# heitorrapela/HalluciDet

Measured on AMD Instinct MI355X. Metric: images/sec train_hallucidet (640x512, batch 8/GPU), higher is better.
Workload: dtype f16; 1 GPU; train_hallucidet.py fasterrcnn LLVIP batch=8 fp16 on 1xMI355X (BASELINE configs[1]); U-Net resnet34 fwd+bwd, 3 frozen Faster R-CNN R50-FPN passes @300x300 (one batched evaluation of 24 images: trunk, RPN, RoI heads, NMS for all three; the RGB / IR passes' LOSS VALUES, which the reference computes and discards, are not evaluated), loss scaling, value clip 0.5, Adam; global_batch=8, image=1x512x640 IR + 3x512x640 RGB, batch_per_gpu=8, parallelism=dp1

## Files before the change

hallucidet_amd/csrc/detection.hip:

```cpp
#include "hd_common.h"
#pragma clang fp contract(off)

namespace {

__device__ __forceinline__ float box_iou_dev(const float* a, const float* b) {
  float area_a = (a[2] - a[0]) * (a[3] - a[1]);
  float area_b = (b[2] - b[0]) * (b[3] - b[1]);
  float xx1 = fmaxf(a[0], b[0]), yy1 = fmaxf(a[1], b[1]);
  float xx2 = fminf(a[2], b[2]), yy2 = fminf(a[3], b[3]);
  float w = fmaxf(0.f, xx2 - xx1), h = fmaxf(0.f, yy2 - yy1);
  float inter = w * h;
  return inter / (area_a + area_b - inter);
}

__global__ void nms_mask_kernel(const float* __restrict__ boxes, const int* __restrict__ counts, int nmax, float thr,
                                uint64_t* __restrict__ mask) {
  const int b = blockIdx.z;
  const int n = counts[b];
  const int row0 = blockIdx.y * 64, col0 = blockIdx.x * 64;
  if (row0 >= n || col0 >= n || blockIdx.x < blockIdx.y) return;
  const int cb = (nmax + 63) / 64;
  __shared__ float cbx[64 * 4];
  const float* bb = boxes + (size_t)b * nmax * 4;
  int t = threadIdx.x;
  int ncol = min(64, n - col0);
  if (t < ncol) {
    cbx[t * 4 + 0] = bb[(col0 + t) * 4 + 0];
    cbx[t * 4 + 1] = bb[(col0 + t) * 4 + 1];
    cbx[t * 4 + 2] = bb[(col0 + t) * 4 + 2];
    cbx[t * 4 + 3] = bb[(col0 + t) * 4 + 3];
  }
  __syncthreads();
  int i = row0 + t;
  if (i < n) {
    float me[4] = {bb[i * 4], bb[i * 4 + 1], bb[i * 4 + 2], bb[i * 4 + 3]};
    uint64_t m = 0;
    int start = (row0 == col0) ? t + 1 : 0;
    for (int j = start; j < ncol; ++j)
      if (box_iou_dev(me, cbx + j * 4) > thr) m |= (1ull << j);
    mask[((size_t)b * nmax + i) * cb + blockIdx.x] = m;
  }
}

__global__ __launch_bounds__(256) void nms_reduce_kernel(const uint64_t* __restrict__ mask, const int* __restrict__ counts, int nmax,
                                                         uint8_t* __restrict__ keep, int max_keep, const int64_t* __restrict__ order,
                                                         int64_t* __restrict__ pick, int pick_n, int64_t* __restrict__ picked) {
  constexpr int MAXW = 4;
  __shared__ uint64_t remv[MAXW * 64];
  __shared__ uint64_t part[4][MAXW * 64];
  __shared__ uint64_t s_keepbits;
  __shared__ int s_kept;
  const int b = blockIdx.x;
  const int n = counts[b];
  const int cb = (nmax + 63) / 64;
  const int tid = threadIdx.x, lane = tid & 63, wave = tid >> 6;
  const uint64_t* mb = mask + (size_t)b * nmax * cb;
  uint8_t* kb = keep + (size_t)b * nmax;
  const int nchunks = (n + 63) / 64;
  for (int i = tid; i < MAXW * 64; i += 256) remv[i] = 0;
  if (tid == 0) s_kept = 0;
  if (pick)
    for (int i = tid; i < pick_n; i += 256) pick[(size_t)b * pick_n + i] = order[(size_t)b * nmax];
  __syncthreads();
  for (int c = 0; c < nchunks; ++c) {
    if (s_kept >= max_keep) {
      for (int i = c * 64 + tid; i < n; i += 256) kb[i] = 0;
      break;
    }
    const int lim = min(64, n - c * 64);
    if (wave == 0) {
      const int i = c * 64 + lane;
      const uint64_t diag = (i < n) ? mb[(size_t)i * cb + c] : 0;
      const unsigned dlo = (unsigned)diag, dhi = (unsigned)(diag >> 32);
      uint64_t alive = ~remv[c];
      if (lim < 64) alive &= (1ull << lim) - 1ull;
      alive = ((uint64_t)(unsigned)__builtin_amdgcn_readfirstlane((unsigned)(alive >> 32)) << 32) |
              (uint64_t)(unsigned)__builtin_amdgcn_readfirstlane((unsigned)alive);
      uint64_t keepbits = 0;
      for (int it = 0; it < 64 && alive; ++it) {
        const int j = __builtin_amdgcn_readfirstlane(__builtin_ctzll(alive));
        keepbits |= (1ull << j);
        const uint64_t dj = ((uint64_t)(unsigned)__builtin_amdgcn_readlane(dhi, j) << 32) | (uint64_t)(unsigned)__builtin_amdgcn_readlane(dlo, j);
        alive &= ~dj;
        alive &= ~(1ull << j);
      }
      if (i < n) kb[i] = (uint8_t)((keepbits >> lane) & 1ull);
      if (pick && ((keepbits >> lane) & 1ull)) {
        const int pos = s_kept + __popcll(keepbits & ((1ull << lane) - 1ull));
        if (pos < pick_n) pick[(size_t)b * pick_n + pos] = order[(size_t)b * nmax + i];
      }
      if (lane == 0) {
        s_keepbits = keepbits;
        s_kept += __popcll(keepbits);
      }
    }
    __syncthreads();
    const uint64_t keepbits = s_keepbits;
    const int nw = nchunks - (c + 1);
    if (nw > 0) {
      for (int wb = 0; wb < nw; wb += 64) {
        const int w = c + 1 + wb + lane;
        const bool act = w < nchunks;
        uint64_t accw = 0;
        for (int jb = wave * 16; jb < lim; jb += 64) {
          uint64_t rws[16];
#pragma unroll
          for (int u = 0; u < 16; ++u) {
            const int j = min(jb + u, lim - 1);
            rws[u] = act ? mb[(size_t)(c * 64 + j) * cb + w] : 0ull;
          }
#pragma unroll
          for (int u = 0; u < 16; ++u)
            if (jb + u < lim && ((keepbits >> (jb + u)) & 1ull)) accw |= rws[u];
        }
        part[wave][wb + lane] = accw;
      }
      __syncthreads();
      for (int i = tid; i < nw; i += 256) remv[c + 1 + i] |= part[0][i] | part[1][i] | part[2][i] | part[3][i];
    }
    __syncthreads();
  }
  if (picked && tid == 0) picked[b] = min(s_kept, pick_n);
}

__global__ __launch_bounds__(256) void nms_prepare_kernel(const float* __restrict__ boxes, const int64_t* __restrict__ idxs,
                                                          const uint8_t* __restrict__ valid, const int64_t* __restrict__ order, int n,
                                                          float* __restrict__ sorted, int* __restrict__ counts) {
  __shared__ float s_max[4];
  __shared__ int s_cnt[4];
  const int b = blockIdx.x, tid = threadIdx.x;
  const float* bb = boxes + (size_t)b * n * 4;
  const uint8_t* vb = valid + (size_t)b * n;
  float m = -INFINITY;
  int cnt = 0;
  for (int i = tid; i < n; i += 256)
    if (vb[i]) {
      const float4 v = *reinterpret_cast<const float4*>(bb + (size_t)i * 4);
      m = fmaxf(fmaxf(m, fmaxf(v.x, v.y)), fmaxf(v.z, v.w));
      ++cnt;
    }
#pragma unroll
  for (int d = 32; d >= 1; d >>= 1) {
    m = fmaxf(m, __shfl_xor(m, d));
    cnt += __shfl_xor(cnt, d);
  }
  if ((tid & 63) == 0) {
    s_max[tid >> 6] = m;
    s_cnt[tid >> 6] = cnt;
  }
  __syncthreads();
  cnt = s_cnt[0] + s_cnt[1] + s_cnt[2] + s_cnt[3];
  m = fmaxf(fmaxf(s_max[0], s_max[1]), fmaxf(s_max[2], s_max[3]));
  const float scale = (cnt > 0 ? m : 0.f) + 1.f;
  if (tid == 0) counts[b] = cnt;
  for (int j = tid; j < n; j += 256) {
    const int64_t c = order[(size_t)b * n + j];
    const float off = (float)idxs[(size_t)b * n + c] * scale;
    float4 v = *reinterpret_cast<const float4*>(bb + (size_t)c * 4);
    v.x += off; v.y += off; v.z += off; v.w += off;
    *reinterpret_cast<float4*>(sorted + ((size_t)b * n + j) * 4) = v;
  }
}

struct NmsSegs {
  int off[9];
  int L, S;
};

__global__ __launch_bounds__(256) void nms_seg_prepare_kernel(const float* __restrict__ boxes, const uint8_t* __restrict__ valid, int n, NmsSegs sg,
                                                              float* __restrict__ sorted, int64_t* __restrict__ order, int* __restrict__ counts) {
  __shared__ float s_max[4];
  __shared__ int s_cnt[4];
  __shared__ int s_wsum[4];
  const int b = blockIdx.x, tid = threadIdx.x, lane = tid & 63, wave = tid >> 6;
  const float* bb = boxes + (size_t)b * n * 4;
  const uint8_t* vb = valid + (size_t)b * n;
  float m = -INFINITY;
  int cnt = 0;
  for (int i = tid; i < n; i += 256)
    if (vb[i]) {
      const float4 v = *reinterpret_cast<const float4*>(bb + (size_t)i * 4);
      m = fmaxf(fmaxf(m, fmaxf(v.x, v.y)), fmaxf(v.z, v.w));
      ++cnt;
    }
#pragma unroll
  for (int d = 32; d >= 1; d >>= 1) {
    m = fmaxf(m, __shfl_xor(m, d));
    cnt += __shfl_xor(cnt, d);
  }
  if (lane == 0) {
    s_max[wave] = m;
    s_cnt[wave] = cnt;
  }
  __syncthreads();
  cnt = s_cnt[0] + s_cnt[1] + s_cnt[2] + s_cnt[3];
  m = fmaxf(fmaxf(s_max[0], s_max[1]), fmaxf(s_max[2], s_max[3]));
  const float scale = (cnt > 0 ? m : 0.f) + 1.f;
  for (int l = 0; l < sg.L; ++l) {
    const int lo = sg.off[l], hi = sg.off[l + 1];
    const float off = (float)l * scale;
    float* so = sorted + ((size_t)b * sg.L + l) * sg.S * 4;
    int64_t* oo = order + ((size_t)b * sg.L + l) * sg.S;
    int base = 0;
    for (int c0 = lo; c0 < hi; c0 += 256) {
      const int i = c0 + tid;
      const bool v = i < hi && vb[i];
      const uint64_t bal = __ballot(v);
      const int before = __popcll(bal & ((1ull << lane) - 1ull));
      __syncthreads();
      if (lane == 0) s_wsum[wave] = __popcll(bal);
      __syncthreads();
      int wbase = 0;
      for (int w = 0; w < wave; ++w) wbase += s_wsum[w];
      if (v) {
        const int r = base + wbase + before;
        float4 bx = *reinterpret_cast<const float4*>(bb + (size_t)i * 4);
        bx.x += off; bx.y += off; bx.z += off; bx.w += off;
        *reinterpret_cast<float4*>(so + (size_t)r * 4) = bx;
        oo[r] = i;
      }
      base += s_wsum[0] + s_wsum[1] + s_wsum[2] + s_wsum[3];
    }
    if (tid == 0) counts[b * sg.L + l] = base;
  }
}

__global__ __launch_bounds__(256) void nms_seg_merge_kernel(const float* __restrict__ scores, const int64_t* __restrict__ pick_seg,
                                                            const int64_t* __restrict__ picked_seg, int n, int pick_n_seg, NmsSegs sg, int top_k,
                                                            int64_t* __restrict__ pick, int64_t* __restrict__ picked) {
  extern __shared__ float s_sc[];
  const int b = blockIdx.x / sg.L, l = blockIdx.x % sg.L;
  const float* sb = scores + (size_t)b * n;
  int cnt[8], total = 0;
  for (int q = 0; q < sg.L; ++q) {
    cnt[q] = (int)picked_seg[b * sg.L + q];
    total += cnt[q];
    const int64_t* pq = pick_seg + ((size_t)b * sg.L + q) * pick_n_seg;
    for (int r = threadIdx.x; r < cnt[q]; r += 256) s_sc[q * pick_n_seg + r] = sb[pq[r]];
  }
  __syncthreads();
  const int64_t* pk = pick_seg + (size_t)blockIdx.x * pick_n_seg;
  for (int r = threadIdx.x; r < cnt[l]; r += 256) {
    const float sc = s_sc[l * pick_n_seg + r];
    int rank = r;
    for (int q = 0; q < sg.L; ++q) {
      if (q == l) continue;
      const float* a = s_sc + q * pick_n_seg;
      int lo = 0, hi = cnt[q];
      if (q < l) {
        while (lo < hi) { const int mid = (lo + hi) >> 1; if (a[mid] >= sc) lo = mid + 1; else hi = mid; }
      } else {
        while (lo < hi) { const int mid = (lo + hi) >> 1; if (a[mid] > sc) lo = mid + 1; else hi = mid; }
      }
      rank += lo;
    }
    if (rank < top_k) pick[(size_t)b * top_k + rank] = pk[r];
  }
  if (l == 0) {
    int64_t best = 0;
    float bs = -INFINITY;
    bool any = false;
    for (int q = 0; q < sg.L; ++q)
      if (cnt[q] > 0 && (!any || s_sc[q * pick_n_seg] > bs)) {
        any = true;
        bs = s_sc[q * pick_n_seg];
        best = pick_seg[((size_t)b * sg.L + q) * pick_n_seg];
      }
    const int have = total < top_k ? total : top_k;
    for (int r = have + threadIdx.x; r < top_k; r += 256) pick[(size_t)b * top_k + r] = best;
    if (threadIdx.x == 0) picked[b] = have;
  }
}

__global__ void box_iou_kernel(const float* __restrict__ gt, int G, const float* __restrict__ boxes, int A, float* __restrict__ iou) {
  const int64_t total = (int64_t)G * A;
  for (int64_t i = (int64_t)blockIdx.x * blockDim.x + threadIdx.x; i < total; i += (int64_t)gridDim.x * blockDim.x) {
    int a = (int)(i % A), g = (int)(i / A);
    iou[i] = box_iou_dev(gt + g * 4, boxes + (size_t)a * 4);
  }
}

__global__ void box_iou_batched_kernel(const float* __restrict__ gt, int G, const float* __restrict__ boxes, int A, int N,
                                       long boxes_stride, float* __restrict__ iou) {
  const int64_t total = (int64_t)N * G * A;
  for (int64_t i = (int64_t)blockIdx.x * blockDim.x + threadIdx.x; i < total; i += (int64_t)gridDim.x * blockDim.x) {
    int a = (int)(i % A);
    int64_t q = i / A;
    int g = (int)(q % G);
    int n = (int)(q / G);
    iou[i] = box_iou_dev(gt + ((size_t)n * G + g) * 4, boxes + (size_t)n * boxes_stride + (size_t)a * 4);
  }
}


template <bool DESC>
__device__ __forceinline__ void radix_find_digit(const int* hist, int remaining, uint32_t prefix, int shift, uint32_t* s_prefix,
                                                 int* s_remaining) {
  if (threadIdx.x >= 64) return;
  const int l = threadIdx.x;
  int h[4], tot = 0;
#pragma unroll
  for (int j = 0; j < 4; ++j) {
    h[j] = hist[DESC ? 255 - (4 * l + j) : 4 * l + j];
    tot += h[j];
  }
  int incl = tot;
#pragma unroll
  for (int d = 1; d < 64; d <<= 1) {
    const int t = __shfl_up(incl, d);
    if (l >= d) incl += t;
  }
  const int excl = incl - tot;
  const bool hit = excl < remaining && remaining <= incl;
  const bool fallback = l == 63 && incl < remaining;
  if (hit || fallback) {
    int cum = excl, j = 0;
    for (; j < 3; ++j) {
      if (cum + h[j] >= remaining) break;
      cum += h[j];
    }
    const int bin = DESC ? 255 - (4 * l + j) : 4 * l + j;
    *s_prefix = prefix | ((uint32_t)bin << shift);
    *s_remaining = remaining - cum;
  }
}

__device__ __forceinline__ uint32_t order_key(float f) {
  if (f != f) return 0xFFFFFFFFu;
  uint32_t u = __float_as_uint(f == 0.f ? 0.f : f);
  return (u & 0x80000000u) ? ~u : (u | 0x80000000u);
}

struct TopkSegs {
  int nseg;
  int seg_off[8], n[8], k[8], out_off[8];
};

__global__ __launch_bounds__(1024) void topk_select_kernel(const float* __restrict__ scores, long row_stride, TopkSegs segs,
                                                           int64_t* __restrict__ out, long out_stride) {
  const int seg_off = segs.seg_off[blockIdx.y], n = segs.n[blockIdx.y], k = segs.k[blockIdx.y], out_off = segs.out_off[blockIdx.y];
  const int64_t idx_add = seg_off;
  __shared__ int hist[256];
  __shared__ uint32_t s_prefix;
  __shared__ int s_remaining;
  __shared__ int s_wave_g[16], s_wave_e[16];
  __shared__ uint64_t s_pair[4096];
  const int tid = threadIdx.x, lane = tid & 63, wave = tid >> 6;
  const float* row = scores + (size_t)blockIdx.x * row_stride + seg_off;
  int64_t* orow = out + (size_t)blockIdx.x * out_stride + out_off;
  int P = 1;
  while (P < k) P <<= 1;
  if (k >= n) {
    for (int i = tid; i < n; i += 1024) s_pair[i] = ((uint64_t)order_key(row[i]) << 32) | (uint32_t)~i;
  } else {
    uint32_t prefix = 0, mask = 0;
    int remaining = k;
    for (int pass = 0; pass < 4; ++pass) {
      const int shift = 24 - 8 * pass;
      if (tid < 256) hist[tid] = 0;
      __syncthreads();
      for (int i = tid; i < n; i += 1024) {
        const uint32_t u = order_key(row[i]);
        if ((u & mask) == prefix) atomicAdd(&hist[(u >> shift) & 255], 1);
      }
      __syncthreads();
      radix_find_digit<true>(hist, remaining, prefix, shift, &s_prefix, &s_remaining);
      __syncthreads();
      prefix = s_prefix;
      remaining = s_remaining;
      mask |= 255u << shift;
      __syncthreads();
    }
    const uint32_t T = prefix;
    int base_g = 0, base_e = 0;
    for (int i0 = 0; i0 < n; i0 += 1024) {
      const int i = i0 + tid;
      const uint32_t u = i < n ? order_key(row[i]) : 0u;
      const bool gt = i < n && u > T, eq = i < n && u == T;
      const uint64_t bg = __ballot(gt), be = __ballot(eq);
      const uint64_t below = (1ull << lane) - 1ull;
      if (lane == 0) {
        s_wave_g[wave] = __popcll(bg);
        s_wave_e[wave] = __popcll(be);
      }
      __syncthreads();
      int g_before = base_g + __popcll(bg & below), e_before = base_e + __popcll(be & below);
      int tot_g = 0, tot_e = 0;
#pragma unroll
      for (int w = 0; w < 16; ++w) {
        if (w < wave) {
          g_before += s_wave_g[w];
          e_before += s_wave_e[w];
        }
        tot_g += s_wave_g[w];
        tot_e += s_wave_e[w];
      }
      if (gt || (eq && e_before < remaining)) s_pair[g_before + min(e_before, remaining)] = ((uint64_t)u << 32) | (uint32_t)~i;
      base_g += tot_g;
      base_e += tot_e;
      __syncthreads();
    }
  }
  for (int i = k + tid; i < P; i += 1024) s_pair[i] = 0;
  __syncthreads();
  for (int size = 2; size <= P; size <<= 1) {
    for (int stride = size >> 1; stride > 0; stride >>= 1) {
      for (int t = tid; t < (P >> 1); t += 1024) {
        const int lo = 2 * t - (t & (stride - 1));
        const int hi = lo + stride;
        const bool desc = (lo & size) == 0;
        const uint64_t a = s_pair[lo], b = s_pair[hi];
        if ((a < b) == desc) {
          s_pair[lo] = b;
          s_pair[hi] = a;
        }
      }
      __syncthreads();
    }
  }
  for (int i = tid; i < k; i += 1024) orow[i] = (int64_t)(uint32_t)~(uint32_t)s_pair[i] + idx_add;
}

__device__ __forceinline__ float4 decode_clip_dev(const float* c, const float* b, float iwx, float iwy, float iww, float iwh, float xclip,
                                                  float img_h, float img_w) {
  const float w = b[2] - b[0], h = b[3] - b[1];
  const float cx = b[0] + 0.5f * w, cy = b[1] + 0.5f * h;
  const float dx = c[0] * iwx, dy = c[1] * iwy;
  float dw = c[2] * iww, dh = c[3] * iwh;
  dw = dw > xclip ? xclip : dw;
  dh = dh > xclip ? xclip : dh;
  const float pcx = dx * w + cx, pcy = dy * h + cy;
  const float pw = expf(dw) * w, ph = expf(dh) * h;
  float4 o;
  o.x = pcx - 0.5f * pw;
  o.y = pcy - 0.5f * ph;
  o.z = pcx + 0.5f * pw;
  o.w = pcy + 0.5f * ph;
  o.x = o.x < 0.f ? 0.f : (o.x > img_w ? img_w : o.x);
  o.z = o.z < 0.f ? 0.f : (o.z > img_w ? img_w : o.z);
  o.y = o.y < 0.f ? 0.f : (o.y > img_h ? img_h : o.y);
  o.w = o.w < 0.f ? 0.f : (o.w > img_h ? img_h : o.w);
  return o;
}

__global__ void rpn_decode_filter_kernel(const float* __restrict__ deltas, const float* __restrict__ obj, const float* __restrict__ anchors,
                                         const int64_t* __restrict__ top, int N, int A, int K, float xclip, float img_h, float img_w,
                                         float min_size, float score_thresh, float* __restrict__ boxes, float* __restrict__ prob,
                                         uint8_t* __restrict__ valid) {
  const int j = blockIdx.x * blockDim.x + threadIdx.x;
  if (j >= N * K) return;
  const int n = j / K;
  const int64_t a = top[j];
  const float4 o = decode_clip_dev(deltas + ((size_t)n * A + a) * 4, anchors + (size_t)a * 4, 1.f, 1.f, 1.f, 1.f, xclip, img_h, img_w);
  const float x = obj[(size_t)n * A + a];
  const float p = 1.f / (1.f + expf(-x));
  *reinterpret_cast<float4*>(boxes + (size_t)j * 4) = o;
  prob[j] = p;
  valid[j] = ((o.z - o.x) >= min_size) && ((o.w - o.y) >= min_size) && (p >= score_thresh);
}

__global__ void roi_decode_clip_kernel(const float* __restrict__ codes, const float* __restrict__ rois, long roi_stride, int R, int K,
                                       float wx, float wy, float ww, float wh, float xclip, float img_h, float img_w,
                                       float* __restrict__ boxes) {
  const int j = blockIdx.x * blockDim.x + threadIdx.x;
  if (j >= R * K) return;
  const int r = j / K;
  *reinterpret_cast<float4*>(boxes + (size_t)j * 4) = decode_clip_dev(codes + (size_t)j * 4, rois + (size_t)r * roi_stride, wx, wy, ww, wh, xclip,
                                                                      img_h, img_w);
}

__global__ void roi_postprocess_kernel(const float* __restrict__ logits, const float* __restrict__ codes, const float* __restrict__ rois,
                                       long roi_stride, const int64_t* __restrict__ counts, int R, int C, int S, float wx, float wy, float ww,
                                       float wh, float xclip, float img_h, float img_w, float score_thresh, float min_size,
                                       float* __restrict__ boxes, float* __restrict__ scores, uint8_t* __restrict__ valid) {
  const int K = C - 1;
  const int j = blockIdx.x * blockDim.x + threadIdx.x;
  if (j >= R * K) return;
  const int r = j / K, k = j - r * K + 1;
  const bool real = (r % S) < (int)counts[r / S];
  float4 o = make_float4(0.f, 0.f, 0.f, 0.f);
  float p = 0.f;
  bool v = false;
  if (real) {
    const float* lr = logits + (size_t)r * C;
    float mx = lr[0];
    for (int c = 1; c < C; ++c) mx = fmaxf(mx, lr[c]);
    float se = 0.f;
    for (int c = 0; c < C; ++c) se += expf(lr[c] - mx);
    p = expf(lr[k] - mx) / se;
    o = decode_clip_dev(codes + ((size_t)r * C + k) * 4, rois + (size_t)r * roi_stride, wx, wy, ww, wh, xclip, img_h, img_w);
    v = (p > score_thresh) && ((o.z - o.x) >= min_size) && ((o.w - o.y) >= min_size);
  }
  *reinterpret_cast<float4*>(boxes + (size_t)j * 4) = o;
  scores[j] = p;
  valid[j] = v;
}

__global__ void roi_samples_finish_kernel(const int64_t* __restrict__ sel, int R, const float* __restrict__ comb, const int64_t* __restrict__ lab,
                                          const int64_t* __restrict__ matched, const float* __restrict__ gt, const uint8_t* __restrict__ gvalid,
                                          int T, int G, float wx, float wy, float ww, float wh, float* __restrict__ rois,
                                          int64_t* __restrict__ labels, float* __restrict__ reg_t) {
  const int r = blockIdx.x * blockDim.x + threadIdx.x;
  if (r >= R) return;
  const int64_t s = sel[r];
  if (s < 0) {
    rois[(size_t)r * 5 + 0] = (float)(-s - 1);
    rois[(size_t)r * 5 + 1] = rois[(size_t)r * 5 + 2] = rois[(size_t)r * 5 + 3] = rois[(size_t)r * 5 + 4] = 0.f;
    labels[r] = -1;
    *reinterpret_cast<float4*>(reg_t + (size_t)r * 4) = make_float4(0.f, 0.f, 0.f, 0.f);
    return;
  }
  const int n = (int)(s / T);
  const float4 b = *reinterpret_cast<const float4*>(comb + (size_t)s * 4);
  bool has_gt = false;
  for (int g = 0; g < G; ++g) has_gt = has_gt || gvalid[(size_t)n * G + g];
  const int64_t m = matched[s];
  float4 rg = make_float4(0.f, 0.f, 0.f, 0.f);
  if (has_gt) rg = *reinterpret_cast<const float4*>(gt + ((size_t)n * G + (m > 0 ? m : 0)) * 4);
  rois[(size_t)r * 5 + 0] = (float)n;
  rois[(size_t)r * 5 + 1] = b.x;
  rois[(size_t)r * 5 + 2] = b.y;
  rois[(size_t)r * 5 + 3] = b.z;
  rois[(size_t)r * 5 + 4] = b.w;
  labels[r] = lab[s];
  const float ew = b.z - b.x, eh = b.w - b.y;
  const float ecx = b.x + 0.5f * ew, ecy = b.y + 0.5f * eh;
  const float gw = rg.z - rg.x, gh = rg.w - rg.y;
  const float gcx = rg.x + 0.5f * gw, gcy = rg.y + 0.5f * gh;
  float4 t;
  t.x = wx * (gcx - ecx) / ew;
// ... 115 lines not shown
    const int i = i0 + tid;
    const bool mem = i < A && member(i);
    const uint32_t u = mem ? key_of(i) : 0xFFFFFFFFu;
    const bool lt = mem && u < T, eq = mem && u == T;
    const uint64_t be = __ballot(eq);
    if (lane == 0) s_wave_e[wave] = __popcll(be);
    __syncthreads();
    int e_before = base_e + __popcll(be & ((1ull << lane) - 1ull));
    int tot_e = 0;
#pragma unroll
    for (int w = 0; w < 16; ++w) {
      if (w < wave) e_before += s_wave_e[w];
      tot_e += s_wave_e[w];
    }
    if (i < A) out[i] = (lt || (eq && e_before < remaining)) ? 1 : 0;
    base_e += tot_e;
    __syncthreads();
  }
}

__global__ __launch_bounds__(1024) void sample_pos_neg_kernel(const int64_t* __restrict__ labels, const int32_t* __restrict__ keys, int A,
                                                              int batch_size, int cap_pos, uint8_t* __restrict__ pos_sel,
                                                              uint8_t* __restrict__ neg_sel, int64_t* __restrict__ counts, int use_lds) {
  __shared__ int hist[256];
  __shared__ uint32_t s_prefix;
  __shared__ int s_remaining;
  __shared__ int s_wave_l[16], s_wave_e[16];
  __shared__ int s_P, s_N;
  extern __shared__ uint32_t s_dyn[];
  const int n = blockIdx.x, tid = threadIdx.x;
  const int64_t* lb = labels + (size_t)n * A;
  const int32_t* kb = keys + (size_t)n * A;
  uint32_t* lk = use_lds ? s_dyn : nullptr;
  uint8_t* lc = use_lds ? reinterpret_cast<uint8_t*>(s_dyn + A) : nullptr;
  if (tid == 0) s_P = s_N = 0;
  __syncthreads();
  int p = 0, q = 0;
  for (int i = tid; i < A; i += 1024) {
    const int64_t l = lb[i];
    p += l >= 1;
    q += l == 0;
    if (use_lds) {
      lk[i] = (uint32_t)kb[i];
      lc[i] = l >= 1 ? 1 : (l == 0 ? 0 : 2);
    }
  }
#pragma unroll
  for (int d = 32; d >= 1; d >>= 1) {
    p += __shfl_xor(p, d);
    q += __shfl_xor(q, d);
  }
  if ((tid & 63) == 0) {
    atomicAdd(&s_P, p);
    atomicAdd(&s_N, q);
  }
  __syncthreads();
  const int P = s_P, Nn = s_N;
  const int num_pos = min(P, cap_pos);
  const int num_neg = min(Nn, batch_size - num_pos);
  if (tid == 0) {
    counts[(size_t)n * 2 + 0] = num_pos;
    counts[(size_t)n * 2 + 1] = num_neg;
  }
  select_smallest_marked(kb, lb, A, true, num_pos, P, pos_sel + (size_t)n * A, hist, &s_prefix, &s_remaining, s_wave_l, s_wave_e, lk, lc);
  __syncthreads();
  select_smallest_marked(kb, lb, A, false, num_neg, Nn, neg_sel + (size_t)n * A, hist, &s_prefix, &s_remaining, s_wave_l, s_wave_e, lk, lc);
}


__global__ __launch_bounds__(1024) void match_best_kernel(const float* __restrict__ gt, const uint8_t* __restrict__ gvalid, int G,
                                                          const float* __restrict__ boxes, int A, long boxes_stride,
                                                          float* __restrict__ best) {
  const int ng = blockIdx.x;
  const int n = ng / G;
  __shared__ float red[16];
  float m = -1.f;
  if (gvalid[ng]) {
    const float g4[4] = {gt[(size_t)ng * 4 + 0], gt[(size_t)ng * 4 + 1], gt[(size_t)ng * 4 + 2], gt[(size_t)ng * 4 + 3]};
    const float* bb = boxes + (size_t)n * boxes_stride;
    for (int a = threadIdx.x; a < A; a += 1024) m = fmaxf(m, box_iou_dev(g4, bb + (size_t)a * 4));
  }
#pragma unroll
  for (int d = 32; d >= 1; d >>= 1) m = fmaxf(m, __shfl_xor(m, d));
  if ((threadIdx.x & 63) == 0) red[threadIdx.x >> 6] = m;
  __syncthreads();
  if (threadIdx.x == 0) {
    float r = red[0];
#pragma unroll
    for (int w = 1; w < 16; ++w) r = fmaxf(r, red[w]);
    best[ng] = r;
  }
}

__global__ __launch_bounds__(256) void match_assign_kernel(const float* __restrict__ gt, const uint8_t* __restrict__ gvalid,
                                                           const int64_t* __restrict__ glabels, int G, const float* __restrict__ boxes,
                                                           int A, int N, long boxes_stride, float high, float low,
                                                           const float* __restrict__ best, float wx, float wy, float ww, float wh,
                                                           int want_reg, int64_t* __restrict__ matched, int64_t* __restrict__ labels,
                                                           float* __restrict__ reg_t) {
  extern __shared__ float s_gt[];
  const int n = blockIdx.y;
  float* s_best = s_gt + G * 4;
  float* s_valid = s_best + G;
  for (int i = threadIdx.x; i < G * 4; i += 256) s_gt[i] = gt[(size_t)n * G * 4 + i];
  for (int i = threadIdx.x; i < G; i += 256) {
    s_best[i] = best ? best[n * G + i] : 0.f;
    s_valid[i] = gvalid[n * G + i] ? 1.f : 0.f;
  }
  __syncthreads();
  const int a = blockIdx.x * 256 + threadIdx.x;
  if (a >= A) return;
  const float* bp = boxes + (size_t)n * boxes_stride + (size_t)a * 4;
  const float b4[4] = {bp[0], bp[1], bp[2], bp[3]};
  float vmax = -INFINITY;
  int imax = 0;
  bool is_best = false, has_gt = false;
  for (int g = 0; g < G; ++g) {
    const bool v = s_valid[g] != 0.f;
    has_gt = has_gt || v;
    const float iou = v ? box_iou_dev(s_gt + g * 4, b4) : -1.f;
    if (iou > vmax) {
      vmax = iou;
      imax = g;
    }
    if (best && v && iou == s_best[g]) is_best = true;
  }
  int64_t m = imax;
  if (vmax < low) m = -1;
  else if (vmax < high) m = -2;
  if (is_best) m = imax;
  const size_t o = (size_t)n * A + a;
  matched[o] = m;
  if (labels) {
    int64_t lab = m >= 0 ? (glabels ? glabels[(size_t)n * G + m] : 1) : (m == -1 ? 0 : -1);
    labels[o] = has_gt ? lab : 0;
  }
  if (want_reg) {
    const float* r = s_gt + (m > 0 ? (int)m : 0) * 4;
    const float ew = b4[2] - b4[0], eh = b4[3] - b4[1];
    const float ecx = b4[0] + 0.5f * ew, ecy = b4[1] + 0.5f * eh;
    const float gw = r[2] - r[0], gh = r[3] - r[1];
    const float gcx = r[0] + 0.5f * gw, gcy = r[1] + 0.5f * gh;
    float4 t;
    t.x = wx * (gcx - ecx) / ew;
    t.y = wy * (gcy - ecy) / eh;
    t.z = ww * logf(gw / ew);
    t.w = wh * logf(gh / eh);
    *reinterpret_cast<float4*>(reg_t + o * 4) = t;
  }
}

}

extern "C" int hd_box_iou_batched(const float* gt, int G, const float* boxes, int A, int N, int shared_boxes, float* iou, void* stream) {
  HD_CHECK_ARG(gt && boxes && iou && G >= 0 && A >= 0 && N >= 0, "hd_box_iou_batched: bad args");
  if (G == 0 || A == 0 || N == 0) return HD_OK;
  int64_t total = (int64_t)N * G * A;
  int g = (int)((total + 255) / 256);
  if (g > 8192) g = 8192;
  hipLaunchKernelGGL(box_iou_batched_kernel, dim3(g), dim3(256), 0, (hipStream_t)stream, gt, G, boxes, A, N,
                     shared_boxes ? 0l : (long)A * 4, iou);
  HD_CHECK_LAUNCH();
  return HD_OK;
}


extern "C" int hd_rpn_decode_filter(const float* deltas, const float* objectness, const float* anchors, const int64_t* top, int N, int A, int K,
                                    float bbox_xform_clip, float img_h, float img_w, float min_size, float score_thresh, float* boxes,
                                    float* prob, uint8_t* valid, void* stream) {
  HD_CHECK_ARG(deltas && objectness && anchors && top && boxes && prob && valid && N >= 0 && A >= 0 && K >= 0, "hd_rpn_decode_filter: bad args");
  if (N * K == 0) return HD_OK;
  hipLaunchKernelGGL(rpn_decode_filter_kernel, dim3((N * K + 255) / 256), dim3(256), 0, (hipStream_t)stream, deltas, objectness, anchors, top, N,
                     A, K, bbox_xform_clip, img_h, img_w, min_size, score_thresh, boxes, prob, valid);
  HD_CHECK_LAUNCH();
  return HD_OK;
}

extern "C" int hd_roi_decode_clip(const float* codes, const float* rois, long roi_stride, int R, int K, const float* coder_weights,
                                  float bbox_xform_clip, float img_h, float img_w, float* boxes, void* stream) {
  HD_CHECK_ARG(codes && rois && coder_weights && boxes && R >= 0 && K >= 0 && roi_stride >= 4, "hd_roi_decode_clip: bad args");
  if (R * K == 0) return HD_OK;
  hipLaunchKernelGGL(roi_decode_clip_kernel, dim3((R * K + 255) / 256), dim3(256), 0, (hipStream_t)stream, codes, rois, roi_stride, R, K,
                     1.0f / coder_weights[0], 1.0f / coder_weights[1], 1.0f / coder_weights[2], 1.0f / coder_weights[3], bbox_xform_clip, img_h,
                     img_w, boxes);
  HD_CHECK_LAUNCH();
  return HD_OK;
}

extern "C" int hd_roi_postprocess(const float* class_logits, const float* box_regression, const float* rois, long roi_stride, const int64_t* counts,
                                  int R, int C, int S, const float* coder_weights, float bbox_xform_clip, float img_h, float img_w, float score_thresh,
                                  float min_size, float* boxes, float* scores, uint8_t* valid, void* stream) {
  HD_CHECK_ARG(class_logits && box_regression && rois && counts && coder_weights && boxes && scores && valid && R >= 0 && C >= 2 && S > 0 &&
               roi_stride >= 4, "hd_roi_postprocess: bad args");
  if (R == 0) return HD_OK;
  const int total = R * (C - 1);
  hipLaunchKernelGGL(roi_postprocess_kernel, dim3((total + 255) / 256), dim3(256), 0, (hipStream_t)stream, class_logits, box_regression, rois,
                     roi_stride, counts, R, C, S, 1.0f / coder_weights[0], 1.0f / coder_weights[1], 1.0f / coder_weights[2], 1.0f / coder_weights[3],
                     bbox_xform_clip, img_h, img_w, score_thresh, min_size, boxes, scores, valid);
  HD_CHECK_LAUNCH();
  return HD_OK;
}

extern "C" int hd_roi_samples_finish(const int64_t* sel, int R, const float* comb, const int64_t* lab, const int64_t* matched, const float* gt,
                                     const uint8_t* gvalid, int T, int G, const float* coder_weights, float* rois, int64_t* labels, float* reg_t,
                                     void* stream) {
  HD_CHECK_ARG(R >= 0 && T > 0 && G > 0 && coder_weights, "hd_roi_samples_finish: bad args");
  if (R == 0) return HD_OK;
  HD_CHECK_ARG(sel && comb && lab && matched && gt && gvalid && rois && labels && reg_t, "hd_roi_samples_finish: null pointer");
  hipLaunchKernelGGL(roi_samples_finish_kernel, dim3((R + 255) / 256), dim3(256), 0, (hipStream_t)stream, sel, R, comb, lab, matched, gt, gvalid, T,
                     G, coder_weights[0], coder_weights[1], coder_weights[2], coder_weights[3], rois, labels, reg_t);
  HD_CHECK_LAUNCH();
  return HD_OK;
}

extern "C" int hd_roi_samples_padded(const uint8_t* pos_sel, const uint8_t* neg_sel, const float* comb, const int64_t* lab, const int64_t* matched,
                                     const float* gt, const uint8_t* gvalid, int N, int T, int G, int S, const float* coder_weights, float* rois,
                                     int64_t* labels, float* reg_t, int64_t* counts, void* stream) {
  HD_CHECK_ARG(pos_sel && neg_sel && comb && lab && matched && gt && gvalid && coder_weights && rois && labels && reg_t && counts && N > 0 &&
               T > 0 && G > 0 && S > 0, "hd_roi_samples_padded: bad args");
  hipLaunchKernelGGL(roi_samples_padded_kernel, dim3(N), dim3(256), 0, (hipStream_t)stream, pos_sel, neg_sel, comb, lab, matched, gt, gvalid, T, G, S,
                     coder_weights[0], coder_weights[1], coder_weights[2], coder_weights[3], rois, labels, reg_t, counts);
  HD_CHECK_LAUNCH();
  return HD_OK;
}

extern "C" int hd_roi_levels(const float* boxes, long stride, int R, float canonical_scale, float canonical_level, float eps, int k_min, int k_max,
                             int* levels, void* stream) {
  HD_CHECK_ARG(R >= 0 && stride >= 4 && k_max >= k_min && canonical_scale > 0.f, "hd_roi_levels: bad args");
  if (R == 0) return HD_OK;
  HD_CHECK_ARG(boxes && levels, "hd_roi_levels: null pointer");
  hipLaunchKernelGGL(roi_levels_kernel, dim3((R + 255) / 256), dim3(256), 0, (hipStream_t)stream, boxes, stride, R, 1.0f / canonical_scale,
                     canonical_level, eps, (float)k_min, (float)k_max, levels);
  HD_CHECK_LAUNCH();
  return HD_OK;
}

extern "C" int hd_sample_pos_neg(const int64_t* labels, const int32_t* keys, int N, int A, int batch_size, int cap_pos, uint8_t* pos_sel,
                                 uint8_t* neg_sel, int64_t* counts, void* stream) {
  HD_CHECK_ARG(N >= 0 && A >= 0 && batch_size > 0 && cap_pos >= 0 && cap_pos <= batch_size, "hd_sample_pos_neg: bad args");
  if (N == 0 || A == 0) return HD_OK;
  HD_CHECK_ARG(labels && keys && pos_sel && neg_sel && counts, "hd_sample_pos_neg: null pointer");
  const size_t need = (size_t)A * 4 + (((size_t)A + 3) & ~(size_t)3);
  const int use_lds = need <= 150 * 1024 ? 1 : 0;
  hipLaunchKernelGGL(sample_pos_neg_kernel, dim3(N), dim3(1024), use_lds ? need : 0, (hipStream_t)stream, labels, keys, A, batch_size, cap_pos,
                     pos_sel, neg_sel, counts, use_lds);
  HD_CHECK_LAUNCH();
  return HD_OK;
}

extern "C" int hd_topk_select_rows(const float* scores, int B, long row_stride, const int* seg_sizes, int nseg, int k, int64_t* out,
                                   long out_stride, void* stream) {
  HD_CHECK_ARG(scores && out && seg_sizes && B >= 0 && nseg >= 1 && nseg <= 8 && k >= 1, "hd_topk_select_rows: bad args (1 <= nseg <= 8)");
  TopkSegs sg;
  sg.nseg = nseg;
  int off = 0, ooff = 0;
  for (int i = 0; i < nseg; ++i) {
    const int n = seg_sizes[i], kk = k < n ? k : n;
    HD_CHECK_ARG(n >= 1 && kk <= 4096, "hd_topk_select_rows: segments must be non-empty, at most 4096 selected entries each (k=%d, n=%d)", k, n);
    sg.seg_off[i] = off; sg.n[i] = n; sg.k[i] = kk; sg.out_off[i] = ooff;
    off += n;
    ooff += kk;
  }
  if (B == 0) return HD_OK;
  hipLaunchKernelGGL(topk_select_kernel, dim3(B, nseg), dim3(1024), 0, (hipStream_t)stream, scores, row_stride, sg, out, out_stride);
  HD_CHECK_LAUNCH();
  return HD_OK;
}

extern "C" int hd_match_targets(const float* gt, const uint8_t* gvalid, const int64_t* glabels, int G, const float* boxes, int A, int N,
                                int shared_boxes, float high, float low, int allow_low_quality, const float* coder_weights,
                                float* best_ws, int64_t* matched, int64_t* labels, float* reg_t, void* stream) {
  HD_CHECK_ARG(gt && gvalid && boxes && matched && G >= 1 && G <= 2048 && A >= 0 && N >= 0, "hd_match_targets: bad args (1 <= G <= 2048)");
  HD_CHECK_ARG(!allow_low_quality || best_ws, "hd_match_targets: allow_low_quality needs the [N*G] float workspace");
  HD_CHECK_ARG((reg_t == nullptr) == (coder_weights == nullptr), "hd_match_targets: reg_t and coder_weights go together");
  if (A == 0 || N == 0) return HD_OK;
  hipStream_t s = (hipStream_t)stream;
  const long stride = shared_boxes ? 0l : (long)A * 4;
  if (allow_low_quality)
    hipLaunchKernelGGL(match_best_kernel, dim3(N * G), dim3(1024), 0, s, gt, gvalid, G, boxes, A, stride, best_ws);
  const float* w = coder_weights;
  hipLaunchKernelGGL(match_assign_kernel, dim3((A + 255) / 256, N), dim3(256), (size_t)G * 6 * sizeof(float), s, gt, gvalid, glabels, G, boxes,
                     A, N, stride, high, low, allow_low_quality ? (const float*)best_ws : (const float*)nullptr, w ? w[0] : 1.f, w ? w[1] : 1.f,
                     w ? w[2] : 1.f, w ? w[3] : 1.f, reg_t ? 1 : 0, matched, labels, reg_t);
  HD_CHECK_LAUNCH();
  return HD_OK;
}

extern "C" int hd_nms_sorted_batched(const float* boxes, const int* counts, int B, int nmax, float iou_thr, uint64_t* mask_ws,
                                     uint8_t* keep, void* stream) {
  return hd_nms_sorted_batched_topk(boxes, counts, B, nmax, iou_thr, mask_ws, keep, 0x7fffffff, stream);
}

extern "C" int hd_nms_sorted_batched_topk(const float* boxes, const int* counts, int B, int nmax, float iou_thr, uint64_t* mask_ws,
                                          uint8_t* keep, int max_keep, void* stream) {
  HD_CHECK_ARG(boxes && counts && mask_ws && keep && B > 0 && nmax > 0 && nmax <= 16384 && max_keep > 0, "hd_nms_sorted_batched: bad args (nmax<=16384)");
  hipStream_t s = (hipStream_t)stream;
  int cb = (nmax + 63) / 64;
  hipLaunchKernelGGL(nms_mask_kernel, dim3(cb, cb, B), dim3(64), 0, s, boxes, counts, nmax, iou_thr, mask_ws);
  hipLaunchKernelGGL(nms_reduce_kernel, dim3(B), dim3(256), 0, s, (const uint64_t*)mask_ws, counts, nmax, keep, max_keep,
                     (const int64_t*)nullptr, (int64_t*)nullptr, 0, (int64_t*)nullptr);
  HD_CHECK_LAUNCH();
  return HD_OK;
}

extern "C" int hd_batched_nms_pick(const float* boxes, const int64_t* idxs, const uint8_t* valid, const int64_t* order, int B, int n,
                                   float iou_thr, int top_n, float* sorted_ws, int* counts_ws, uint64_t* mask_ws, uint8_t* keep_ws,
                                   int64_t* pick, int64_t* picked, void* stream) {
  HD_CHECK_ARG(boxes && idxs && valid && order && sorted_ws && counts_ws && mask_ws && keep_ws && pick && picked && B > 0 && n > 0 &&
               n <= 16384 && top_n > 0, "hd_batched_nms_pick: bad args (n<=16384)");
  hipStream_t s = (hipStream_t)stream;
  const int cb = (n + 63) / 64;
  hipLaunchKernelGGL(nms_prepare_kernel, dim3(B), dim3(256), 0, s, boxes, idxs, valid, order, n, sorted_ws, counts_ws);
  hipLaunchKernelGGL(nms_mask_kernel, dim3(cb, cb, B), dim3(64), 0, s, (const float*)sorted_ws, (const int*)counts_ws, n, iou_thr, mask_ws);
  hipLaunchKernelGGL(nms_reduce_kernel, dim3(B), dim3(256), 0, s, (const uint64_t*)mask_ws, (const int*)counts_ws, n, keep_ws, top_n, order, pick,
                     top_n < n ? top_n : n, picked);
  HD_CHECK_LAUNCH();
  return HD_OK;
}

extern "C" int hd_batched_nms_pick_segments(const float* boxes, const float* scores, const uint8_t* valid, int B, int n, const int* seg_sizes,
                                            int L, float iou_thr, int top_n, float* sorted_ws, int64_t* order_ws, int* counts_ws,
                                            uint64_t* mask_ws, uint8_t* keep_ws, int64_t* pick_ws, int64_t* picked_seg, int64_t* pick,
                                            int64_t* picked, void* stream) {
  HD_CHECK_ARG(boxes && scores && valid && seg_sizes && sorted_ws && order_ws && counts_ws && mask_ws && keep_ws && pick_ws && picked_seg && pick && picked &&
               B > 0 && n > 0 && L >= 1 && L <= 8 && top_n > 0, "hd_batched_nms_pick_segments: bad args (<= 8 segments)");
  NmsSegs sg;
  sg.L = L;
  sg.S = 1;
  sg.off[0] = 0;
  for (int l = 0; l < L; ++l) {
    HD_CHECK_ARG(seg_sizes[l] > 0, "hd_batched_nms_pick_segments: empty segment");
    sg.off[l + 1] = sg.off[l] + seg_sizes[l];
    if (seg_sizes[l] > sg.S) sg.S = seg_sizes[l];
  }
  for (int l = L + 1; l < 9; ++l) sg.off[l] = sg.off[L];
  HD_CHECK_ARG(sg.off[L] == n && sg.S <= 16384, "hd_batched_nms_pick_segments: segment sizes must add up to n");
  hipStream_t s = (hipStream_t)stream;
  const int S = sg.S, cb = (S + 63) / 64, pick_n = top_n < S ? top_n : S;
  hipLaunchKernelGGL(nms_seg_prepare_kernel, dim3(B), dim3(256), 0, s, boxes, valid, n, sg, sorted_ws, order_ws, counts_ws);
  hipLaunchKernelGGL(nms_mask_kernel, dim3(cb, cb, B * L), dim3(64), 0, s, (const float*)sorted_ws, (const int*)counts_ws, S, iou_thr, mask_ws);
  hipLaunchKernelGGL(nms_reduce_kernel, dim3(B * L), dim3(256), 0, s, (const uint64_t*)mask_ws, (const int*)counts_ws, S, keep_ws, top_n,
                     (const int64_t*)order_ws, pick_ws, pick_n, picked_seg);
  const int top_k = top_n < n ? top_n : n;
  hipLaunchKernelGGL(nms_seg_merge_kernel, dim3(B * L), dim3(256), (size_t)L * pick_n * sizeof(float), s, scores, (const int64_t*)pick_ws,
                     (const int64_t*)picked_seg, n, pick_n, sg, top_k, pick, picked);
  HD_CHECK_LAUNCH();
  return HD_OK;
}

extern "C" int hd_box_iou(const float* gt, int G, const float* boxes, int A, float* iou, void* stream) {
  HD_CHECK_ARG(gt && boxes && iou && G >= 0 && A >= 0, "hd_box_iou: bad args");
  if (G == 0 || A == 0) return HD_OK;
  int64_t total = (int64_t)G * A;
  int g = (int)((total + 255) / 256);
  if (g > 4096) g = 4096;
  hipLaunchKernelGGL(box_iou_kernel, dim3(g), dim3(256), 0, (hipStream_t)stream, gt, G, boxes, A, iou);
  HD_CHECK_LAUNCH();
  return HD_OK;
}
```

Baseline: 828.2 images/s.

## Stage NMS masks and top-k keys in LDS, triangular mask grid, split segment prepare

The NMS mask kernel now launches only the upper-triangular block grid instead of a full square with early exits. The reduce kernel can stage the upper-triangle suppression mask in LDS and process the chunks with a ballot-based in-wave resolve plus parallel atomicOr updates, replacing repeated global reads. Top-k selection caches order keys in dynamic LDS across the radix passes, and segment preparation can run one 1024-thread block per segment. All new paths are on by default behind environment knobs, and they use far more LDS per block, which may reduce occupancy.

```diff
diff --git a/hallucidet_amd/csrc/detection.hip b/hallucidet_amd/csrc/detection.hip
--- a/hallucidet_amd/csrc/detection.hip
+++ b/hallucidet_amd/csrc/detection.hip
@@ -17,9 +17,15 @@
                                 uint64_t* __restrict__ mask) {
   const int b = blockIdx.z;
   const int n = counts[b];
-  const int row0 = blockIdx.y * 64, col0 = blockIdx.x * 64;
-  if (row0 >= n || col0 >= n || blockIdx.x < blockIdx.y) return;
   const int cb = (nmax + 63) / 64;
+  int rowblk = 0, rem = blockIdx.x;
+  while (rem >= cb - rowblk) {
+    rem -= cb - rowblk;
+    ++rowblk;
+  }
+  const int colblk = rowblk + rem;
+  const int row0 = rowblk * 64, col0 = colblk * 64;
+  if (row0 >= n || col0 >= n) return;
   __shared__ float cbx[64 * 4];
   const float* bb = boxes + (size_t)b * nmax * 4;
   int t = threadIdx.x;
@@ -38,18 +44,24 @@
     int start = (row0 == col0) ? t + 1 : 0;
     for (int j = start; j < ncol; ++j)
       if (box_iou_dev(me, cbx + j * 4) > thr) m |= (1ull << j);
-    mask[((size_t)b * nmax + i) * cb + blockIdx.x] = m;
-  }
-}
+    mask[((size_t)b * nmax + i) * cb + colblk] = m;
+  }
+}
+
+constexpr int NMS_MAXW = 4;
+constexpr size_t NMS_STATIC_LDS = (size_t)NMS_MAXW * 64 * 8 * 5 + 16;
+constexpr size_t nms_lds_bytes(int cb) { return (size_t)512 * cb * (cb + 1) / 2; }
 
 __global__ __launch_bounds__(256) void nms_reduce_kernel(const uint64_t* __restrict__ mask, const int* __restrict__ counts, int nmax,
                                                          uint8_t* __restrict__ keep, int max_keep, const int64_t* __restrict__ order,
-                                                         int64_t* __restrict__ pick, int pick_n, int64_t* __restrict__ picked) {
-  constexpr int MAXW = 4;
+                                                         int64_t* __restrict__ pick, int pick_n, int64_t* __restrict__ picked, int use_lds) {
+  constexpr int MAXW = NMS_MAXW;
   __shared__ uint64_t remv[MAXW * 64];
   __shared__ uint64_t part[4][MAXW * 64];
   __shared__ uint64_t s_keepbits;
   __shared__ int s_kept;
+  extern __shared__ uint64_t s_mask[];
+  static_assert(sizeof(remv) + sizeof(part) + 16 == NMS_STATIC_LDS, "NMS_STATIC_LDS is what the launcher's limit subtracts");
   const int b = blockIdx.x;
   const int n = counts[b];
   const int cb = (nmax + 63) / 64;
@@ -59,8 +71,93 @@
   const int nchunks = (n + 63) / 64;
   for (int i = tid; i < MAXW * 64; i += 256) remv[i] = 0;
   if (tid == 0) s_kept = 0;
-  if (pick)
+  if (pick && !use_lds)
     for (int i = tid; i < pick_n; i += 256) pick[(size_t)b * pick_n + i] = order[(size_t)b * nmax];
+  if (use_lds) {
+    uint64_t* s_keepw = part[0];
+    uint64_t* s_before = part[1];
+    for (int i = tid; i < nchunks; i += 256) s_keepw[i] = 0;
+    uint64_t* tri = s_mask + nchunks * 64;
+    int lg = 0;
+    while ((1 << lg) < nchunks) ++lg;
+    const int total = n << lg;
+    for (int f0 = tid; f0 < total; f0 += 256 * 16) {
+      uint64_t v[16];
+#pragma unroll
+      for (int u = 0; u < 16; ++u) {
+        const int f = f0 + u * 256, i = f >> lg, w = f & ((1 << lg) - 1);
+        v[u] = (i < n && w < nchunks && w >= (i >> 6)) ? mb[(size_t)i * cb + w] : 0ull;
+      }
+#pragma unroll
+      for (int u = 0; u < 16; ++u) {
+        const int f = f0 + u * 256, i = f >> lg, w = f & ((1 << lg) - 1), c = i >> 6;
+        if (i < n && w < nchunks && w >= c) {
+          if (w == c) s_mask[i] = v[u];
+          else tri[64 * (c * (nchunks - 1) - c * (c - 1) / 2) + (i & 63) * (nchunks - 1 - c) + (w - c - 1)] = v[u];
+        }
+      }
+    }
+    __syncthreads();
+    int kept = 0;
+    for (int c = 0; c < nchunks; ++c) {
+      if (kept >= max_keep) break;
+      const int lim = min(64, n - c * 64);
+      if (wave == 0) {
+        const int i = c * 64 + lane;
+        const uint64_t diag = (i < n) ? s_mask[i] : 0;
+        const unsigned dlo = (unsigned)diag, dhi = (unsigned)(diag >> 32);
+        uint64_t alive = ~remv[c];
+        if (lim < 64) alive &= (1ull << lim) - 1ull;
+        alive = ((uint64_t)(unsigned)__builtin_amdgcn_readfirstlane((unsigned)(alive >> 32)) << 32) |
+                (uint64_t)(unsigned)__builtin_amdgcn_readfirstlane((unsigned)alive);
+        uint64_t act = __ballot((diag & alive) != 0) & alive;
+        act = ((uint64_t)(unsigned)__builtin_amdgcn_readfirstlane((unsigned)(act >> 32)) << 32) |
+              (uint64_t)(unsigned)__builtin_amdgcn_readfirstlane((unsigned)act);
+        while (act) {
+          const int j = __builtin_amdgcn_readfirstlane(__builtin_ctzll(act));
+          const uint64_t dj = ((uint64_t)(unsigned)__builtin_amdgcn_readlane(dhi, j) << 32) | (uint64_t)(unsigned)__builtin_amdgcn_readlane(dlo, j);
+          alive &= ~dj;
+          act &= ~(dj | (1ull << j));
+        }
+        const uint64_t keepbits = alive;
+        if (lane == 0) {
+          s_keepw[c] = keepbits;
+          s_before[c] = (uint64_t)kept;
+        }
+      }
+      __syncthreads();
+      const uint64_t keepbits = s_keepw[c];
+      kept += __popcll(keepbits);
+      const int nw = nchunks - 1 - c;
+      if (lane < nw) {
+        const uint64_t* tc = tri + 64 * (c * (nchunks - 1) - c * (c - 1) / 2) + lane;
+        const int j0 = __builtin_amdgcn_readfirstlane(wave) * 16;
+        uint64_t rws[16], accw = 0;
+#pragma unroll
+        for (int u = 0; u < 16; ++u) rws[u] = tc[min(j0 + u, lim - 1) * nw];
+#pragma unroll
+        for (int u = 0; u < 16; ++u)
+          if (j0 + u < lim && ((keepbits >> (j0 + u)) & 1ull)) accw |= rws[u];
+        if (accw) atomicOr((unsigned long long*)&remv[c + 1 + lane], (unsigned long long)accw);
+      }
+      __syncthreads();
+    }
+    const int have = min(kept, pick_n);
+    for (int i = tid; i < n; i += 256) {
+      const int c = i >> 6, l = i & 63;
+      const uint64_t kw = s_keepw[c];
+      const bool k = (kw >> l) & 1ull;
+      kb[i] = (uint8_t)k;
+      if (pick && k) {
+        const int pos = (int)s_before[c] + __popcll(kw & ((1ull << l) - 1ull));
+        if (pos < pick_n) pick[(size_t)b * pick_n + pos] = order[(size_t)b * nmax + i];
+      }
+    }
+    if (pick)
+      for (int i = have + tid; i < pick_n; i += 256) pick[(size_t)b * pick_n + i] = order[(size_t)b * nmax];
+    if (picked && tid == 0) picked[b] = have;
+    return;
+  }
   __syncthreads();
   for (int c = 0; c < nchunks; ++c) {
     if (s_kept >= max_keep) {
@@ -167,17 +264,20 @@
   int L, S;
 };
 
-__global__ __launch_bounds__(256) void nms_seg_prepare_kernel(const float* __restrict__ boxes, const uint8_t* __restrict__ valid, int n, NmsSegs sg,
-                                                              float* __restrict__ sorted, int64_t* __restrict__ order, int* __restrict__ counts) {
-  __shared__ float s_max[4];
-  __shared__ int s_cnt[4];
-  __shared__ int s_wsum[4];
-  const int b = blockIdx.x, tid = threadIdx.x, lane = tid & 63, wave = tid >> 6;
+__global__ __launch_bounds__(1024) void nms_seg_prepare_kernel(const float* __restrict__ boxes, const uint8_t* __restrict__ valid, int n, NmsSegs sg,
+                                                               int per_seg, float* __restrict__ sorted, int64_t* __restrict__ order,
+                                                               int* __restrict__ counts) {
+  __shared__ float s_max[16];
+  __shared__ int s_cnt[16];
+  __shared__ int s_wsum[16];
+  const int b = per_seg ? blockIdx.x / sg.L : blockIdx.x, tid = threadIdx.x, lane = tid & 63, wave = tid >> 6;
+  const int nthr = blockDim.x, nwave = nthr >> 6;
+  const int l_lo = per_seg ? blockIdx.x % sg.L : 0, l_hi = per_seg ? l_lo + 1 : sg.L;
   const float* bb = boxes + (size_t)b * n * 4;
   const uint8_t* vb = valid + (size_t)b * n;
   float m = -INFINITY;
   int cnt = 0;
-  for (int i = tid; i < n; i += 256)
+  for (int i = tid; i < n; i += nthr)
     if (vb[i]) {
       const float4 v = *reinterpret_cast<const float4*>(bb + (size_t)i * 4);
       m = fmaxf(fmaxf(m, fmaxf(v.x, v.y)), fmaxf(v.z, v.w));
@@ -193,16 +293,20 @@
     s_cnt[wave] = cnt;
   }
   __syncthreads();
-  cnt = s_cnt[0] + s_cnt[1] + s_cnt[2] + s_cnt[3];
-  m = fmaxf(fmaxf(s_max[0], s_max[1]), fmaxf(s_max[2], s_max[3]));
+  cnt = 0;
+  m = -INFINITY;
+  for (int w = 0; w < nwave; ++w) {
+    cnt += s_cnt[w];
+    m = fmaxf(m, s_max[w]);
+  }
   const float scale = (cnt > 0 ? m : 0.f) + 1.f;
-  for (int l = 0; l < sg.L; ++l) {
+  for (int l = l_lo; l < l_hi; ++l) {
     const int lo = sg.off[l], hi = sg.off[l + 1];
     const float off = (float)l * scale;
     float* so = sorted + ((size_t)b * sg.L + l) * sg.S * 4;
     int64_t* oo = order + ((size_t)b * sg.L + l) * sg.S;
     int base = 0;
-    for (int c0 = lo; c0 < hi; c0 += 256) {
+    for (int c0 = lo; c0 < hi; c0 += nthr) {
       const int i = c0 + tid;
       const bool v = i < hi && vb[i];
       const uint64_t bal = __ballot(v);
@@ -210,8 +314,11 @@
       __syncthreads();
       if (lane == 0) s_wsum[wave] = __popcll(bal);
       __syncthreads();
-      int wbase = 0;
-      for (int w = 0; w < wave; ++w) wbase += s_wsum[w];
+      int wbase = 0, wtot = 0;
+      for (int w = 0; w < nwave; ++w) {
+        if (w < wave) wbase += s_wsum[w];
+        wtot += s_wsum[w];
+      }
       if (v) {
         const int r = base + wbase + before;
         float4 bx = *reinterpret_cast<const float4*>(bb + (size_t)i * 4);
@@ -219,7 +326,7 @@
         *reinterpret_cast<float4*>(so + (size_t)r * 4) = bx;
         oo[r] = i;
       }
-      base += s_wsum[0] + s_wsum[1] + s_wsum[2] + s_wsum[3];
+      base += wtot;
     }
     if (tid == 0) counts[b * sg.L + l] = base;
   }
@@ -335,9 +442,11 @@
   int nseg;
   int seg_off[8], n[8], k[8], out_off[8];
 };
+constexpr size_t TOPK_STATIC_LDS = 34 * 1024;
+constexpr int TOPK_LDS_MAX_N = (int)((160 * 1024 - TOPK_STATIC_LDS) / 4);
 
 __global__ __launch_bounds__(1024) void topk_select_kernel(const float* __restrict__ scores, long row_stride, TopkSegs segs,
-                                                           int64_t* __restrict__ out, long out_stride) {
+                                                           int64_t* __restrict__ out, long out_stride, int lds_cap) {
   const int seg_off = segs.seg_off[blockIdx.y], n = segs.n[blockIdx.y], k = segs.k[blockIdx.y], out_off = segs.out_off[blockIdx.y];
   const int64_t idx_add = seg_off;
   __shared__ int hist[256];
@@ -345,11 +454,24 @@
   __shared__ int s_remaining;
   __shared__ int s_wave_g[16], s_wave_e[16];
   __shared__ uint64_t s_pair[4096];
+  extern __shared__ uint32_t s_key[];
+  static_assert(sizeof(hist) + sizeof(s_wave_g) + sizeof(s_wave_e) + sizeof(s_pair) + 16 <= TOPK_STATIC_LDS, "TOPK_STATIC_LDS");
   const int tid = threadIdx.x, lane = tid & 63, wave = tid >> 6;
   const float* row = scores + (size_t)blockIdx.x * row_stride + seg_off;
   int64_t* orow = out + (size_t)blockIdx.x * out_stride + out_off;
   int P = 1;
   while (P < k) P <<= 1;
+  const bool staged = k < n && n <= lds_cap;
+  if (staged) {
+    for (int i0 = tid; i0 < n; i0 += 1024 * 8) {
+      float f[8];
+#pragma unroll
+      for (int u = 0; u < 8; ++u) f[u] = i0 + u * 1024 < n ? row[i0 + u * 1024] : 0.f;
+#pragma unroll
+      for (int u = 0; u < 8; ++u)
+        if (i0 + u * 1024 < n) s_key[i0 + u * 1024] = order_key(f[u]);
+    }
+  }
   if (k >= n) {
     for (int i = tid; i < n; i += 1024) s_pair[i] = ((uint64_t)order_key(row[i]) << 32) | (uint32_t)~i;
   } else {
@@ -360,7 +482,7 @@
       if (tid < 256) hist[tid] = 0;
       __syncthreads();
       for (int i = tid; i < n; i += 1024) {
-        const uint32_t u = order_key(row[i]);
+        const uint32_t u = staged ? s_key[i] : order_key(row[i]);
         if ((u & mask) == prefix) atomicAdd(&hist[(u >> shift) & 255], 1);
       }
       __syncthreads();
@@ -375,7 +497,7 @@
     int base_g = 0, base_e = 0;
     for (int i0 = 0; i0 < n; i0 += 1024) {
       const int i = i0 + tid;
-      const uint32_t u = i < n ? order_key(row[i]) : 0u;
+      const uint32_t u = i < n ? (staged ? s_key[i] : order_key(row[i])) : 0u;
       const bool gt = i < n && u > T, eq = i < n && u == T;
       const uint64_t bg = __ballot(gt), be = __ballot(eq);
       const uint64_t below = (1ull << lane) - 1ull;
@@ -797,6 +919,11 @@
 
 }
 
+static bool hd_knob_on(const char* name) {
+  const char* v = getenv(name);
+  return !(v && v[0] == '0' && v[1] == 0);
+}
+
 extern "C" int hd_box_iou_batched(const float* gt, int G, const float* boxes, int A, int N, int shared_boxes, float* iou, void* stream) {
   HD_CHECK_ARG(gt && boxes && iou && G >= 0 && A >= 0 && N >= 0, "hd_box_iou_batched: bad args");
   if (G == 0 || A == 0 || N == 0) return HD_OK;
@@ -899,15 +1026,19 @@
   TopkSegs sg;
   sg.nseg = nseg;
   int off = 0, ooff = 0;
+  const int max_stage = hd_knob_on("HD_TOPK_LDS") ? TOPK_LDS_MAX_N : 0;
+  int lds_cap = 0;
   for (int i = 0; i < nseg; ++i) {
     const int n = seg_sizes[i], kk = k < n ? k : n;
     HD_CHECK_ARG(n >= 1 && kk <= 4096, "hd_topk_select_rows: segments must be non-empty, at most 4096 selected entries each (k=%d, n=%d)", k, n);
     sg.seg_off[i] = off; sg.n[i] = n; sg.k[i] = kk; sg.out_off[i] = ooff;
     off += n;
     ooff += kk;
+    if (kk < n && n <= max_stage && n > lds_cap) lds_cap = n;
   }
   if (B == 0) return HD_OK;
-  hipLaunchKernelGGL(topk_select_kernel, dim3(B, nseg), dim3(1024), 0, (hipStream_t)stream, scores, row_stride, sg, out, out_stride);
+  hipLaunchKernelGGL(topk_select_kernel, dim3(B, nseg), dim3(1024), (size_t)lds_cap * 4, (hipStream_t)stream, scores, row_stride, sg, out,
+                     out_stride, lds_cap);
   HD_CHECK_LAUNCH();
   return HD_OK;
 }
@@ -931,6 +1062,15 @@
   return HD_OK;
 }
 
+static void launch_nms_mask_reduce(hipStream_t s, const float* boxes, const int* counts, int nblocks, int nmax, float iou_thr, uint64_t* mask_ws,
+                                   uint8_t* keep, int max_keep, const int64_t* order, int64_t* pick, int pick_n, int64_t* picked) {
+  const int cb = (nmax + 63) / 64;
+  const bool lds = hd_knob_on("HD_NMS_LDS") && nms_lds_bytes(cb) + NMS_STATIC_LDS <= (size_t)160 * 1024;
+  hipLaunchKernelGGL(nms_mask_kernel, dim3(cb * (cb + 1) / 2, 1, nblocks), dim3(64), 0, s, boxes, counts, nmax, iou_thr, mask_ws);
+  hipLaunchKernelGGL(nms_reduce_kernel, dim3(nblocks), dim3(256), lds ? nms_lds_bytes(cb) : 0, s, (const uint64_t*)mask_ws, counts, nmax, keep,
+                     max_keep, order, pick, pick_n, picked, lds ? 1 : 0);
+}
+
 extern "C" int hd_nms_sorted_batched(const float* boxes, const int* counts, int B, int nmax, float iou_thr, uint64_t* mask_ws,
                                      uint8_t* keep, void* stream) {
   return hd_nms_sorted_batched_topk(boxes, counts, B, nmax, iou_thr, mask_ws, keep, 0x7fffffff, stream);
@@ -940,10 +1080,7 @@
                                           uint8_t* keep, int max_keep, void* stream) {
   HD_CHECK_ARG(boxes && counts && mask_ws && keep && B > 0 && nmax > 0 && nmax <= 16384 && max_keep > 0, "hd_nms_sorted_batched: bad args (nmax<=16384)");
   hipStream_t s = (hipStream_t)stream;
-  int cb = (nmax + 63) / 64;
-  hipLaunchKernelGGL(nms_mask_kernel, dim3(cb, cb, B), dim3(64), 0, s, boxes, counts, nmax, iou_thr, mask_ws);
-  hipLaunchKernelGGL(nms_reduce_kernel, dim3(B), dim3(256), 0, s, (const uint64_t*)mask_ws, counts, nmax, keep, max_keep,
-                     (const int64_t*)nullptr, (int64_t*)nullptr, 0, (int64_t*)nullptr);
+  launch_nms_mask_reduce(s, boxes, counts, B, nmax, iou_thr, mask_ws, keep, max_keep, nullptr, nullptr, 0, nullptr);
   HD_CHECK_LAUNCH();
   return HD_OK;
 }
@@ -954,11 +1091,8 @@
   HD_CHECK_ARG(boxes && idxs && valid && order && sorted_ws && counts_ws && mask_ws && keep_ws && pick && picked && B > 0 && n > 0 &&
                n <= 16384 && top_n > 0, "hd_batched_nms_pick: bad args (n<=16384)");
   hipStream_t s = (hipStream_t)stream;
-  const int cb = (n + 63) / 64;
   hipLaunchKernelGGL(nms_prepare_kernel, dim3(B), dim3(256), 0, s, boxes, idxs, valid, order, n, sorted_ws, counts_ws);
-  hipLaunchKernelGGL(nms_mask_kernel, dim3(cb, cb, B), dim3(64), 0, s, (const float*)sorted_ws, (const int*)counts_ws, n, iou_thr, mask_ws);
-  hipLaunchKernelGGL(nms_reduce_kernel, dim3(B), dim3(256), 0, s, (const uint64_t*)mask_ws, (const int*)counts_ws, n, keep_ws, top_n, order, pick,
-                     top_n < n ? top_n : n, picked);
+  launch_nms_mask_reduce(s, sorted_ws, counts_ws, B, n, iou_thr, mask_ws, keep_ws, top_n, order, pick, top_n < n ? top_n : n, picked);
   HD_CHECK_LAUNCH();
   return HD_OK;
 }
@@ -981,11 +1115,12 @@
   for (int l = L + 1; l < 9; ++l) sg.off[l] = sg.off[L];
   HD_CHECK_ARG(sg.off[L] == n && sg.S <= 16384, "hd_batched_nms_pick_segments: segment sizes must add up to n");
   hipStream_t s = (hipStream_t)stream;
-  const int S = sg.S, cb = (S + 63) / 64, pick_n = top_n < S ? top_n : S;
-  hipLaunchKernelGGL(nms_seg_prepare_kernel, dim3(B), dim3(256), 0, s, boxes, valid, n, sg, sorted_ws, order_ws, counts_ws);
-  hipLaunchKernelGGL(nms_mask_kernel, dim3(cb, cb, B * L), dim3(64), 0, s, (const float*)sorted_ws, (const int*)counts_ws, S, iou_thr, mask_ws);
-  hipLaunchKernelGGL(nms_reduce_kernel, dim3(B * L), dim3(256), 0, s, (const uint64_t*)mask_ws, (const int*)counts_ws, S, keep_ws, top_n,
-                     (const int64_t*)order_ws, pick_ws, pick_n, picked_seg);
+  const int S = sg.S, pick_n = top_n < S ? top_n : S;
+  if (hd_knob_on("HD_NMS_SEG_SPLIT"))
+    hipLaunchKernelGGL(nms_seg_prepare_kernel, dim3(B * L), dim3(1024), 0, s, boxes, valid, n, sg, 1, sorted_ws, order_ws, counts_ws);
+  else
+    hipLaunchKernelGGL(nms_seg_prepare_kernel, dim3(B), dim3(256), 0, s, boxes, valid, n, sg, 0, sorted_ws, order_ws, counts_ws);
+  launch_nms_mask_reduce(s, sorted_ws, counts_ws, B * L, S, iou_thr, mask_ws, keep_ws, top_n, order_ws, pick_ws, pick_n, picked_seg);
   const int top_k = top_n < n ? top_n : n;
   hipLaunchKernelGGL(nms_seg_merge_kernel, dim3(B * L), dim3(256), (size_t)L * pick_n * sizeof(float), s, scores, (const int64_t*)pick_ws,
                      (const int64_t*)picked_seg, n, pick_n, sg, top_k, pick, picked);
```

Result: no change. 835.2 images/s, median of 6 (+0.8%).
